# jayleicn/ClipBERT

Measured on NVIDIA H100. Metric: clips/sec fwd+bwd MSRVTT ret (ResNet50+BERT-base), higher is better.
Workload: dtype bf16

## Files before the change

clipbert_b200/csrc/gemm.cu:

```cuda
#include <algorithm>

#include "common.cuh"
#include "host_util.h"

namespace cb {

constexpr int BM = 128;
constexpr int BK = 64;
constexpr int CONSUMER_WARPS = 8;
constexpr int GEMM_THREADS = (CONSUMER_WARPS + 1) * 32;
constexpr int PP_THREADS = 3 * 128;
constexpr int PP_PRODUCER_REGS = 40;
constexpr int PP_CONSUMER_REGS = 232;
constexpr int PP_BAR_TURN = 1;
constexpr int MAX_STAGES = 8;
constexpr int SMEM_LIMIT = 232448;
constexpr int STG_PITCH = 36;
constexpr int STG_WARP_FLOATS = 16 * STG_PITCH;
constexpr int EPI_BYTES = CONSUMER_WARPS * STG_WARP_FLOATS * 4;
constexpr int IN_BOX_BYTES = BM * 64 * 2;

struct GemmEpi {
  const float* scale;
  const float* shift;
  const __nv_bfloat16* residual;
  const __nv_bfloat16* aux;
  int aux_mode;
  int act;
  void* out;
  int64_t out_ld;
  int out_fp32;
  __nv_bfloat16* out2;
  int64_t out2_ld;
  int rowmap, H, W;
  uint32_t drop_thresh;
// ... 179 lines not shown
        for (int j = 0; j < NC / 2; ++j) {
          const float2 a2 = unpack_bf16x2(aux16[j]);
          f[2 * j] *= a2.x;
          f[2 * j + 1] *= a2.y;
        }
        break;
      default: break;
    }
  }
}

struct TileInfo {
  int m0, n0;
};

template <int BN>
__device__ __forceinline__ TileInfo decode_tile(int tile, int tiles_m, int tiles_n) {
  TileInfo t;
  t.m0 = (tile / tiles_n) % tiles_m * BM;
  t.n0 = tile % tiles_n * BN;
  return t;
}

template <int BN, int TA, int TB>
__device__ __forceinline__ void mma_tile(float (&acc)[BN / 2], uint32_t smem0, int stage_bytes, int KCH, int STAGES, int n_iters, int wg,
                                         int lane, int& s, uint32_t& ph, uint64_t* full_bar, uint64_t* empty_bar) {
  using Cfg = GemmCfg<BN>;
  int prev = -1;
  for (int i = 0; i < n_iters; i += KCH) {
    const int nch = min(KCH, n_iters - i);
    mbar_wait(&full_bar[s], ph);
    __syncwarp();
    wgmma_fence();
    wgmma_fence_acc(acc);
    for (int ch = 0; ch < nch; ++ch) {
      const uint32_t a_addr = smem0 + s * stage_bytes + ch * Cfg::STAGE_BYTES + wg * (64 * 128);
      const uint32_t b_addr = smem0 + s * stage_bytes + ch * Cfg::STAGE_BYTES + Cfg::A_BYTES;
// ... 10 lines not shown
    if (prev >= 0) {
      __syncwarp();
      if (lane == 0) mbar_arrive(&empty_bar[prev]);
    }
    prev = s;
    if (++s == STAGES) { s = 0; ph ^= 1; }
  }
  wgmma_wait<0>();
  wgmma_fence_acc(acc);
  if (prev >= 0) {
    __syncwarp();
    if (lane == 0) mbar_arrive(&empty_bar[prev]);
  }
}

template <int BN, int TB>
__device__ __forceinline__ void mma_tile_pp(float (&acc)[2][BN / 2], uint32_t smem0, int stage_bytes, int KCH, int STAGES, int n_iters,
                                            int lane, int& s, uint32_t& ph, uint64_t* full_bar, uint64_t* empty_bar, int pass_bar,
                                            bool in_stage) {
  using Cfg = GemmCfg<BN>;
  int prev = -1;
  for (int i = 0; i < n_iters; i += KCH) {
    const int nch = min(KCH, n_iters - i);
    mbar_wait_unguarded(&full_bar[s], ph);
    __syncwarp();
    wgmma_fence();
    wgmma_fence_acc(acc[0]);
    wgmma_fence_acc(acc[1]);
    for (int ch = 0; ch < nch; ++ch) {
      const uint32_t a_addr = smem0 + s * stage_bytes + ch * Cfg::STAGE_BYTES;
      const uint32_t b_addr = a_addr + Cfg::A_BYTES;
#pragma unroll
      for (int k = 0; k < BK / 16; ++k) {
        const uint64_t bd = TB ? gmma_desc(b_addr + k * 2048, BK * 128, 1024) : gmma_desc(b_addr + k * 32, 16, 1024);
        const uint32_t accum = (i > 0 || ch > 0 || k > 0) ? 1u : 0u;
#pragma unroll
        for (int h = 0; h < 2; ++h) wgmma_bf16<BN, 0, TB>(acc[h], gmma_desc(a_addr + h * (64 * 128) + k * 32, 16, 1024), bd, accum);
      }
    }
    wgmma_commit();
    wgmma_wait<1>();
    wgmma_fence_acc(acc[0]);
    wgmma_fence_acc(acc[1]);
    if (prev >= 0) {
      __syncwarp();
      mbar_arrive_if(&empty_bar[prev], lane == 0);
// ... 25 lines not shown
    const int n = n0 + j * 8 + 2 * (lane & 3);
    if (n < N) {
      if constexpr (STORE) {
        if (r0 < M) *reinterpret_cast<float2*>(obase + static_cast<int64_t>(r0) * out_ld + n) = make_float2(acc[4 * j] * rs0, acc[4 * j + 1] * rs0);
        if (r1 < M) *reinterpret_cast<float2*>(obase + static_cast<int64_t>(r1) * out_ld + n) = make_float2(acc[4 * j + 2] * rs1, acc[4 * j + 3] * rs1);
      } else {
        if (r0 < M) red_add_f32x2(obase + static_cast<int64_t>(r0) * out_ld + n, acc[4 * j] * rs0, acc[4 * j + 1] * rs0);
        if (r1 < M) red_add_f32x2(obase + static_cast<int64_t>(r1) * out_ld + n, acc[4 * j + 2] * rs1, acc[4 * j + 3] * rs1);
      }
    }
  }
}

__device__ __forceinline__ uint32_t swz128(uint32_t box, int r, int q) { return box + r * 128 + ((q ^ (r & 7)) << 4); }

template <int BN, int MODE>
__global__ void __launch_bounds__(PP_THREADS, 1)
    gemm_pingpong_kernel(const __grid_constant__ CUtensorMap tmA, const __grid_constant__ CUtensorMap tmB, const __grid_constant__ CUtensorMap tmR,
                         const __grid_constant__ CUtensorMap tmX, int M, int N, int K, int ntaps, int tap_w, int tap_sign, int tiles_m,
                         int tiles_n, int total_tiles, int STAGES, int KCH, int N_IN, GemmEpi epi) {
  static_assert(MODE != 1 && BN <= 128, "TN / NN tiles of 128 x 64 or 128 x 128");
  using Cfg = GemmCfg<BN>;
  extern __shared__ uint8_t smem_raw[];
  uint8_t* smem = reinterpret_cast<uint8_t*>((reinterpret_cast<uintptr_t>(smem_raw) + 1023) & ~static_cast<uintptr_t>(1023));
  const int stage_bytes = KCH * Cfg::STAGE_BYTES;
  const bool has_res = epi.residual != nullptr, has_aux = epi.aux != nullptr;
  constexpr int IN_TILE_BYTES = (BN / 64) * IN_BOX_BYTES;
  const int in_bytes = (has_res + has_aux) * IN_TILE_BYTES;
  uint8_t* in_base = smem + STAGES * stage_bytes;
  uint8_t* stg_base = in_base + N_IN * in_bytes;
  uint64_t* full_bar = reinterpret_cast<uint64_t*>(stg_base + EPI_BYTES);
  uint64_t* empty_bar = full_bar + MAX_STAGES;
  uint64_t* in_full = empty_bar + MAX_STAGES;
  uint64_t* in_empty = in_full + 2;

  const int warp = __shfl_sync(0xffffffffu, static_cast<int>(threadIdx.x >> 5), 0);
  const int lane = threadIdx.x & 31;
  const int unit = blockIdx.x;
  const int n_units = gridDim.x;
  if (threadIdx.x == 0) dbg_stamp(epi, 0);
  pdl_trigger();
  if (threadIdx.x == 0) {
    tma_prefetch_desc(&tmA);
    tma_prefetch_desc(&tmB);
    if (has_res) tma_prefetch_desc(&tmR);
    if (has_aux) tma_prefetch_desc(&tmX);
    for (int s = 0; s < STAGES; ++s) {
      mbar_init(&full_bar[s], 1);
      mbar_init(&empty_bar[s], 4);
    }
    for (int b = 0; b < 2; ++b) {
      mbar_init(&in_full[b], 1);
      mbar_init(&in_empty[b], 4);
    }
    fence_mbar_init();
  }
  __syncthreads();
  const int kc_per_tap = (K + BK - 1) / BK;
  const int n_iters = ntaps * kc_per_tap;
  const bool in_stage = in_bytes && !N_IN;
  const int tile_stages = (n_iters + KCH - 1) / KCH + (in_stage ? 1 : 0);
  pdl_wait();
  if (threadIdx.x == 0) dbg_stamp(epi, 1);

  if (warp < 4) {
    setmaxnreg_dec<PP_PRODUCER_REGS>();
    if (warp == 0 && lane == 0) {
      constexpr int B_BOXES = (MODE == 0) ? 1 : BN / 64;
      int s = 0;
      uint32_t ph = 0;
      auto load_inputs = [&](int tile) {
        const TileInfo t = decode_tile<BN>(tile, tiles_m, tiles_n);
        uint64_t* bar;
        uint8_t* dst;
        if (N_IN) {
          const int local = (tile - unit) / n_units;
          const int b = N_IN == 2 ? (local & 1) : 0;
          const int uses = N_IN == 2 ? (local >> 1) : local;
          mbar_wait(&in_empty[b], (static_cast<uint32_t>(uses) & 1u) ^ 1u);
          bar = &in_full[local & 1];
          dst = in_base + b * in_bytes;
        } else {
          mbar_wait(&empty_bar[s], ph ^ 1);
          bar = &full_bar[s];
          dst = smem + s * stage_bytes;
          if (++s == STAGES) { s = 0; ph ^= 1; }
        }
        mbar_expect_tx(bar, in_bytes);
        if (has_res) {
#pragma unroll
          for (int j = 0; j < BN / 64; ++j) tma_load_2d(dst + j * IN_BOX_BYTES, &tmR, bar, t.n0 + j * 64, t.m0);
          dst += IN_TILE_BYTES;
        }
        if (has_aux) {
#pragma unroll
          for (int j = 0; j < BN / 64; ++j) tma_load_2d(dst + j * IN_BOX_BYTES, &tmX, bar, t.n0 + j * 64, t.m0);
        }
      };
      int pend = -1;
      for (int tile = unit; tile < total_tiles; tile += n_units) {
        const TileInfo t = decode_tile<BN>(tile, tiles_m, tiles_n);
        const bool inputs_first = tile < unit + N_IN * n_units;
        if (in_bytes && N_IN && inputs_first) load_inputs(tile);
        for (int i = 0; i < n_iters; i += KCH) {
          const int nch = min(KCH, n_iters - i);
          mbar_wait(&empty_bar[s], ph ^ 1);
          mbar_expect_tx(&full_bar[s], nch * Cfg::STAGE_BYTES);
          int tp = 0, kc = i;
          if (ntaps > 1) { tp = i / kc_per_tap; kc = i - tp * kc_per_tap; }
          for (int ch = 0; ch < nch; ++ch) {
            uint8_t* sa = smem + s * stage_bytes + ch * Cfg::STAGE_BYTES;
            uint8_t* sb = sa + Cfg::A_BYTES;
            int shift = 0;
            if (ntaps == 9) shift = tap_sign * ((tp / 3 - 1) * tap_w + (tp % 3 - 1));
            else if (ntaps > 1) shift = tap_sign * tp * tap_w;
            tma_load_2d(sa, &tmA, &full_bar[s], kc * BK, t.m0 + shift);
            if (MODE == 0) {
              tma_load_2d(sb, &tmB, &full_bar[s], tp * K + kc * BK, t.n0);
            } else if (epi.mn3d) {
              tma_load_3d(sb, &tmB, &full_bar[s], 0, kc * BK, (tp * N + t.n0) >> 6);
            } else {
#pragma unroll
              for (int j = 0; j < B_BOXES; ++j) tma_load_2d(sb + j * (BK * 128), &tmB, &full_bar[s], tp * N + t.n0 + j * 64, kc * BK);
            }
            if (++kc == kc_per_tap) { kc = 0; ++tp; }
          }
          if (++s == STAGES) { s = 0; ph ^= 1; }
          if (i == 0 && tile == unit) dbg_stamp(epi, 2);
        }
        if (in_stage) load_inputs(tile);
        if (pend >= 0) load_inputs(pend);
        pend = (in_bytes && N_IN && !inputs_first) ? tile : -1;
      }
      if (pend >= 0) load_inputs(pend);
      dbg_stamp(epi, 3);
    }
    return;
  }

  setmaxnreg_inc<PP_CONSUMER_REGS>();
  const int wg = (warp >> 2) - 1;
  const int wq = warp & 3;
  const uint32_t smem0 = smem_u32(smem);
  const uint64_t dseed = epi.drop_thresh ? drop_seed(epi.seed, epi.seed_off) : 0ull;
  float acc[2][BN / 2];
  int s = 0;
  uint32_t ph = 0;
  auto ring_skip = [&](int n) {
    s += n;
    while (s >= STAGES) { s -= STAGES; ph ^= 1; }
  };
  if (wg == 1) ring_skip(tile_stages);

  const int er = lane & 15, eh = lane >> 4;
  float* stg = reinterpret_cast<float*>(stg_base) + (warp - 4) * STG_WARP_FLOATS;
  const bool has_out2 = epi.out2 != nullptr;
  const bool has_shift = epi.shift != nullptr;
  const bool full = (N & 15) == 0 && epi.scale == nullptr;
  const bool drop = epi.drop_thresh != 0;
  int kind = EK_GENERIC;
  if (full) {
    if (!drop && !has_out2 && !has_aux && (epi.act == CB_ACT_NONE || epi.act == CB_ACT_RELU)) kind = EK_SHIFT_ACT;
    else if (!drop && !has_out2 && !has_shift && has_aux && epi.aux_mode == CB_AUX_RELU_MASK && epi.act == CB_ACT_NONE) kind = EK_RELU_MASK;
    else if (drop && !has_out2 && !has_aux && epi.act == CB_ACT_NONE) kind = EK_DROP_RES;
    else if (!drop && has_out2 && !has_aux && !has_res && epi.act == CB_ACT_GELU_STASH_GRAD) kind = EK_GELU_STASH;
    else if (!drop && !has_out2 && !has_shift && has_aux && epi.aux_mode == CB_AUX_MUL && epi.act == CB_ACT_NONE) kind = EK_AUX_MUL;
  }
  const bool kind_relu = epi.act == CB_ACT_RELU;
  const bool guard = (N & 15) != 0;

  for (int local = wg, tile = unit + wg * n_units; tile < total_tiles; local += 2, tile += 2 * n_units) {
    const TileInfo t = decode_tile<BN>(tile, tiles_m, tiles_n);
    if (local > 0) named_bar_sync(PP_BAR_TURN + wg, 2 * 128);
    const int pass = tile + n_units < total_tiles ? PP_BAR_TURN + (wg ^ 1) : 0;
    mma_tile_pp<BN, MODE != 0>(acc, smem0, stage_bytes, KCH, STAGES, n_iters, lane, s, ph, full_bar, empty_bar, pass, in_stage);

    const uint32_t in_buf = N_IN ? smem_u32(in_base) + (N_IN == 2 ? wg : 0) * in_bytes : smem0 + s * stage_bytes;
    if (in_bytes) {
      if (N_IN) mbar_wait_unguarded(&in_full[wg], static_cast<uint32_t>(local >> 1) & 1u);
      else mbar_wait_unguarded(&full_bar[s], ph);
    }
    int orow_half[2];
#pragma unroll
    for (int h = 0; h < 2; ++h) {
      const int m = t.m0 + h * 64 + wq * 16 + er;
      bool row_ok = m < M;
      int64_t orow = m;
      if (epi.rowmap == CB_ROWMAP_PAD) {
        const int hw = epi.H * epi.W;
        const int img = m / hw;
        const int r = m - img * hw;
        const int y = r / epi.W, x = r - y * epi.W;
        orow = (static_cast<int64_t>(img) * (epi.H + 2) + y + 1) * (epi.W + 2) + x + 1;
      } else if (epi.rowmap == CB_ROWMAP_UNPAD) {
        const int wp = epi.W + 2, hp = epi.H + 2;
// ... 25 lines not shown
        const int64_t orow = h ? orow_half[1] : orow_half[0];
        if (orow < 0 || nb >= N) continue;
        constexpr int NC = 16;
        float f[NC];
        const uint32_t srow = smem_u32(stg + er * STG_PITCH + eh * 16);
#pragma unroll
        for (int j = 0; j < NC / 4; ++j) {
          const uint4 u = lds128(srow + j * 16);
          f[4 * j] = __uint_as_float(u.x); f[4 * j + 1] = __uint_as_float(u.y);
          f[4 * j + 2] = __uint_as_float(u.z); f[4 * j + 3] = __uint_as_float(u.w);
        }
        uint32_t res16[NC / 2], aux16[NC / 2];
        const int tc = sc * 32 + eh * 16;
        const int q = (tc & 63) >> 3;
        if (has_res) {
#pragma unroll
          for (int j = 0; j < 2; ++j) {
            const uint4 u = lds128(swz128(in_buf + (tc >> 6) * IN_BOX_BYTES, wrow + er, q + j));
            res16[4 * j] = u.x; res16[4 * j + 1] = u.y; res16[4 * j + 2] = u.z; res16[4 * j + 3] = u.w;
          }
        }
        if (has_aux) {
#pragma unroll
          for (int j = 0; j < 2; ++j) {
            const uint4 u = lds128(swz128(in_buf + (has_res ? IN_TILE_BYTES : 0) + (tc >> 6) * IN_BOX_BYTES, wrow + er, q + j));
            aux16[4 * j] = u.x; aux16[4 * j + 1] = u.y; aux16[4 * j + 2] = u.z; aux16[4 * j + 3] = u.w;
          }
        }
        float shv[NC];
        if (has_shift) {
#pragma unroll
          for (int j = 0; j < NC; j += 4) {
            float4 s4 = make_float4(0.f, 0.f, 0.f, 0.f);
            if (nb + j + 4 <= N) s4 = __ldg(reinterpret_cast<const float4*>(epi.shift + nb + j));
            shv[j] = s4.x; shv[j + 1] = s4.y; shv[j + 2] = s4.z; shv[j + 3] = s4.w;
          }
        }
        uint32_t o2_16[NC / 2];
        switch (kind) {
          case EK_SHIFT_ACT: epilogue_shift_act<NC>(f, shv, has_shift, res16, has_res, kind_relu); break;
// ... 17 lines not shown
          __nv_bfloat16* o = reinterpret_cast<__nv_bfloat16*>(epi.out) + orow * epi.out_ld + nb;
#pragma unroll
          for (int j = 0; j < 2; ++j)
            if (nb + 8 * j + 8 <= N)
              *reinterpret_cast<uint4*>(o + 8 * j) = make_uint4(pack_bf16x2(f[8 * j], f[8 * j + 1]), pack_bf16x2(f[8 * j + 2], f[8 * j + 3]),
                                                                pack_bf16x2(f[8 * j + 4], f[8 * j + 5]), pack_bf16x2(f[8 * j + 6], f[8 * j + 7]));
        }
        if (has_out2) {
          __nv_bfloat16* o = epi.out2 + orow * epi.out2_ld + nb;
#pragma unroll
          for (int j = 0; j < 2; ++j)
            if (nb + 8 * j + 8 <= N) *reinterpret_cast<uint4*>(o + 8 * j) = make_uint4(o2_16[4 * j], o2_16[4 * j + 1], o2_16[4 * j + 2], o2_16[4 * j + 3]);
        }
      }
    }
    if (in_bytes) {
      __syncwarp();
      if (lane == 0) mbar_arrive(N_IN ? &in_empty[N_IN == 2 ? wg : 0] : &empty_bar[s]);
      if (!N_IN && ++s == STAGES) { s = 0; ph ^= 1; }
    }
    ring_skip(tile_stages);
  }
  if (threadIdx.x == 4 * 32) dbg_stamp(epi, 11);
}

static int g_sm_limit = 0;
static int sm_count_device() {
  static int n = 0;
  if (n == 0) {
    int dev = 0;
    cudaGetDevice(&dev);
    cudaDeviceGetAttribute(&n, cudaDevAttrMultiProcessorCount, dev);
    if (n <= 0) n = 132;
  }
  return n;
}
// ... 29 lines not shown
  const int stage_iters = ceil_div(kiters, p.kch);
  const int cap = staging ? 2 * stage_iters + 1 : (stage_iters + 1 > 2 ? stage_iters + 1 : 2);
  if (p.stages > cap) p.stages = cap;
  return p;
}
static SmemPlan plan_smem(int bn, bool staging, int kiters, int force_kch = 0, int in_bytes = 0) {
  const SmemPlan none = plan_ring(bn, staging, kiters, force_kch, 0, 0);
  if (in_bytes == 0) return none;
  const SmemPlan two = plan_ring(bn, staging, kiters, force_kch, in_bytes, 2);
  if (two.stages >= 2 && two.stages * two.kch >= kiters) return two;
  if (kiters > 4 && none.stages >= 2 && none.kch * none.chunk_bytes >= in_bytes) return none;
  return plan_ring(bn, staging, kiters, force_kch, in_bytes, 1);
}
static int epi_in_bytes(const cb_gemm_desc& d, int bn) {
  return d.mode == CB_GEMM_WGRAD ? 0 : ((d.residual != nullptr) + (d.aux != nullptr)) * (bn / 64) * IN_BOX_BYTES;
}

static int real_splits(int kc, int want) {
  const int sp = want < 1 ? 1 : (want > kc ? kc : want);
  return ceil_div(kc, ceil_div(kc, sp));
}

struct SplitReduceJob {
  float* out;
  const float* ws;
  int64_t out_ld;
  int M, W, S;
};
struct SplitReduce {
  int njobs;
// ... 14 lines not shown
    for (int s = 0; s < J.S; ++s) {
      const float4 a = *reinterpret_cast<const float4*>(p + s * plane);
      v.x += a.x; v.y += a.y; v.z += a.z; v.w += a.w;
    }
    *o = v;
  }
}
static int launch_split_reduce(const SplitReduce& r, cudaStream_t stream, const char* what) {
  int64_t most = 0;
  for (int i = 0; i < r.njobs; ++i) most = std::max(most, static_cast<int64_t>(r.j[i].M) * (r.j[i].W / 4));
  const int gx = static_cast<int>(std::min<int64_t>(1024, (most + 255) / 256));
  launch_k(wgrad_split_reduce_kernel, dim3(gx, r.njobs), 256, 0, stream, r);
  return check_launch(what);
}

template <int BN, int MODE>
static int launch_gemm(const cb_gemm_desc& d, const GemmEpi& epi_in, cudaStream_t stream) {
  GemmEpi epi = epi_in;
  using Cfg = GemmCfg<BN>;
  static bool attr_set = false;
  auto kern = gemm_pingpong_kernel<BN, MODE>;
  if (!attr_set) {
    cudaError_t e = cudaFuncSetAttribute(kern, cudaFuncAttributeMaxDynamicSharedMemorySize, SMEM_LIMIT);
    if (e != cudaSuccess) {
      set_error("cudaFuncSetAttribute(smem=%d): %s", SMEM_LIMIT, cudaGetErrorString(e));
      return CB_ERR_CUDA;
    }
    attr_set = true;
  }
  alignas(64) CUtensorMap ta, tb, tr, tx;
  bool mn3d = false;
  const int tiles_m = ceil_div(d.m, BM), tiles_n = ceil_div(d.n, BN);
  const int total = tiles_m * tiles_n;
  const int kiters = ceil_div(d.k, BK) * d.ntaps;
  bool ok = get_tmap_2d(&ta, d.a, d.k, d.a_rows, d.a_ld, BK, BM);
  if (MODE == 0) {
    ok = ok && get_tmap_2d(&tb, d.b, static_cast<uint64_t>(d.k) * d.ntaps, d.b_rows, d.b_ld, BK, BN);
  } else {
    mn3d = g_mn3d && d.n % 64 == 0 &&
           get_tmap_3d_mn(&tb, d.b, static_cast<uint64_t>(d.n) * d.ntaps, d.b_rows, d.b_ld, BK, BN / 64);
    if (!mn3d) ok = ok && get_tmap_2d(&tb, d.b, static_cast<uint64_t>(d.n) * d.ntaps, d.b_rows, d.b_ld, 64, BK);
  }
  tr = ta;
  tx = ta;
  if (d.residual) ok = ok && get_tmap_2d(&tr, d.residual, d.n, d.m, d.res_ld, 64, BM);
  if (d.aux) ok = ok && get_tmap_2d(&tx, d.aux, d.n, d.m, d.aux_ld, 64, BM);
  if (!ok) return CB_ERR_CUDA;
  epi.mn3d = mn3d ? 1 : 0;
  const int units = sm_count();
  const int grid = total < units ? total : units;
  const int in_bytes = epi_in_bytes(d, BN);
  const SmemPlan sp = plan_smem(BN, true, kiters, (d.reserved >> 8) & 15, in_bytes);
  const int kch = sp.kch, stages = sp.stages;
  if (stages < 2) {
    set_error("cb_gemm: not enough shared memory for a 2-stage pipeline (BN=%d, epilogue %d B + inputs %d B)", BN, sp.epi_bytes,
              in_bytes);
    return CB_ERR_INVALID;
  }
  const int smem_bytes = stages * kch * Cfg::STAGE_BYTES + sp.n_in * in_bytes + sp.epi_bytes + Cfg::BAR_BYTES + 1024;
  launch_gemm_k(kern, grid, PP_THREADS, smem_bytes, stream, ta, tb, tr, tx, d.m, d.n, d.k, d.ntaps, d.tap_w, d.tap_sign, tiles_m,
                tiles_n, total, stages, kch, sp.n_in, epi);
  return check_launch("cb_gemm");
}

struct LaunchCfg {
  int bn, splits;
};

static LaunchCfg choose_config(const cb_gemm_desc& d, int units) {
  const int kc = ceil_div(d.k, BK);
  const bool wgrad = d.mode == CB_GEMM_WGRAD;
  const int block_n = (!wgrad && d.block_n == 256) ? 128 : d.block_n;
  static const int cand[3] = {64, 128, 256};
  LaunchCfg best = {64, 1};
  double best_cost = 1e30;
  for (int c = 0; c < 3; ++c) {
    const int bn = cand[c];
    if (block_n && bn != block_n) continue;
    if (!wgrad && bn == 256) continue;
    if (bn > 64 && d.n <= bn / 2) continue;
    const int64_t base = static_cast<int64_t>(ceil_div(d.m, BM)) * ceil_div(d.n, bn) * (wgrad ? d.ntaps : 1);
    const int max_split = wgrad ? (d.split_k > 0 ? d.split_k : (kc < 32 ? kc : 32)) : 1;
    for (int sp = (wgrad && d.split_k > 0) ? d.split_k : 1; sp <= max_split; ++sp) {
      const int ips = ceil_div(wgrad ? kc : kc * d.ntaps, sp);
      const int real_sp = wgrad ? ceil_div(kc, ips) : 1;
      const int64_t tiles = base * real_sp;
      const double rounds = static_cast<double>((tiles + units - 1) / units);
      const SmemPlan pl = plan_smem(bn, !wgrad, ips, (d.reserved >> 8) & 15, epi_in_bytes(d, bn));
      if (pl.stages < 2) continue;
      const double shallow = (pl.stages * pl.kch < 3 && ips > 2) ? 3.0 : 1.0;
      const double stage_cost = 450.0 + pl.kch * pl.chunk_bytes / 60.0;
      const double main_loop = ceil_div(ips, pl.kch) * stage_cost * shallow;
      double cost;
      if (wgrad) {
        cost = rounds * (main_loop + bn * 24.0) + 2500.0;
      } else {
        const double epi = bn * 30.0;
        const double per_tile = main_loop > 0.5 * (main_loop + epi) ? main_loop : 0.5 * (main_loop + epi);
        cost = rounds * per_tile + 0.5 * epi + 2500.0;
      }
      if (cost < best_cost) {
        best_cost = cost;
        best = {bn, real_sp};
      }
    }
  }
  return best;
}

constexpr int WG_MAX_PROBLEMS = 8;
struct WgradProblem {
  CUtensorMap tmA, tmB;
  float* out;
  const float* scale;
  int64_t out_ld;
  int M, N, K;
  int ntaps, tap_w, tap_sign;
  int iters_per_split, tiles_m, tiles_n;
// ... 242 lines not shown
                         : launch_wgrad_group<64, false>(descs, n, splits, ws, stream, what);
    case 128: return need ? launch_wgrad_group<128, true>(descs, n, splits, ws, stream, what)
                          : launch_wgrad_group<128, false>(descs, n, splits, ws, stream, what);
    case 256: return need ? launch_wgrad_group<256, true>(descs, n, splits, ws, stream, what)
                          : launch_wgrad_group<256, false>(descs, n, splits, ws, stream, what);
    default: set_error("%s: block_n must be 0, 64, 128 or 256 (got %d)", what, bn); return CB_ERR_INVALID;
  }
}

}

extern "C" void cb_debug_gemm_timeline(void* device_buf) { cb::g_gemm_timeline = static_cast<long long*>(device_buf); }
extern "C" void cb_debug_gemm_mn3d(int on) { cb::g_mn3d = on ? 1 : 0; }
extern "C" void cb_debug_gemm_occ2(int, double) {}
extern "C" void cb_debug_gemm_sm_limit(int n) { cb::g_sm_limit = n > 0 ? n : 0; }

extern "C" int cb_gemm(const cb_gemm_desc* dp, void* stream_v) {
  using namespace cb;
  CB_REQUIRE(dp != nullptr, "cb_gemm: null descriptor");
  const cb_gemm_desc& d = *dp;
  cudaStream_t stream = static_cast<cudaStream_t>(stream_v);
  CB_REQUIRE(d.a && d.b && d.out, "cb_gemm: null operand pointer");
  CB_REQUIRE(d.m > 0 && d.n > 0 && d.k > 0, "cb_gemm: empty problem m=%d n=%d k=%d", d.m, d.n, d.k);
  CB_REQUIRE(d.ntaps == 1 || d.ntaps == 9 || (d.ntaps == 4 && d.mode == CB_GEMM_TN),
             "cb_gemm: ntaps must be 1, 9 (3x3 conv) or 4 (row taps, TN only) (got %d)", d.ntaps);
  CB_REQUIRE(d.mode == CB_GEMM_TN || d.mode == CB_GEMM_WGRAD || d.mode == CB_GEMM_NN, "cb_gemm: bad mode %d", d.mode);
  CB_REQUIRE(d.dropout_p >= 0.0f && d.dropout_p <= 1.0f, "cb_gemm: dropout_p %g outside [0, 1]", d.dropout_p);

  GemmEpi epi;
  epi.scale = d.scale;
// ... 24 lines not shown
    const bool nn = d.mode == CB_GEMM_NN;
    CB_REQUIRE(d.n % 8 == 0, "cb_gemm(TN): n must be a multiple of 8 (got %d)", d.n);
    CB_REQUIRE(d.k % 8 == 0, "cb_gemm(TN): k must be a multiple of 8 (got %d)", d.k);
    CB_REQUIRE(d.out_ld % 8 == 0, "cb_gemm(TN): out_ld must be a multiple of 8");
    CB_REQUIRE(!d.residual || d.res_ld % 8 == 0, "cb_gemm(TN): res_ld must be a multiple of 8");
    CB_REQUIRE(!d.aux || d.aux_ld % 8 == 0, "cb_gemm(TN): aux_ld must be a multiple of 8");
    CB_REQUIRE((reinterpret_cast<uintptr_t>(d.residual) & 15) == 0, "cb_gemm(TN): residual must be 16-byte aligned");
    CB_REQUIRE((reinterpret_cast<uintptr_t>(d.aux) & 15) == 0, "cb_gemm(TN): aux must be 16-byte aligned");
    CB_REQUIRE(!d.out2 || d.out2_ld % 8 == 0, "cb_gemm(TN): out2_ld must be a multiple of 8");
    CB_REQUIRE(!(d.out2 && d.out_fp32), "cb_gemm(TN): out2 requires a bf16 primary output");
    CB_REQUIRE(d.rowmap == CB_ROWMAP_NONE || (d.map_h > 0 && d.map_w > 0), "cb_gemm: rowmap needs map_h/map_w");
    CB_REQUIRE(d.ntaps == 1 || d.tap_w > 2, "cb_gemm: tap modes need tap_w (padded row pitch in pixels)");
    CB_REQUIRE(d.block_n == 0 || d.block_n == 64 || d.block_n == 128 || d.block_n == 256, "cb_gemm: block_n must be 0, 64, 128 or 256 (got %d)",
               d.block_n);
    const LaunchCfg lc = choose_config(d, sm_count());
    switch (lc.bn) {
      case 64: return nn ? launch_gemm<64, 2>(d, epi, stream) : launch_gemm<64, 0>(d, epi, stream);
      case 128: return nn ? launch_gemm<128, 2>(d, epi, stream) : launch_gemm<128, 0>(d, epi, stream);
      default: CB_REQUIRE(false, "cb_gemm: no tile width for block_n %d", d.block_n);
    }
  } else {
    const int rc = check_wgrad_desc(d, "cb_gemm(WGRAD)");
    if (rc != CB_OK) return rc;
    const LaunchCfg lc = choose_config(d, plan_sm_count());
    return launch_wgrad(&d, 1, lc.bn, lc.splits, stream, "cb_gemm");
  }
  return CB_ERR_INVALID;
}

extern "C" int cb_gemm_wgrad_group(const cb_gemm_desc* descs, int n, void* stream_v) {
// ... 36 lines not shown
```

clipbert_b200/ops.py:

```python
import ctypes

import torch

from . import _lib as L
from ._lib import (ACT_GELU, ACT_GELU_STASH_GRAD, ACT_NONE, ACT_RELU, ACT_TANH, AUX_GELU_GRAD, AUX_MUL, AUX_NONE,
                   AUX_RELU_MASK, AUX_TANH_GRAD, CB_GEMM_TN, CB_GEMM_WGRAD, ROWMAP_NONE, ROWMAP_PAD, ROWMAP_UNPAD)

CB_GEMM_NN = 2
_c = ctypes
_vp, _i, _i64, _f, _u64 = _c.c_void_p, _c.c_int, _c.c_int64, _c.c_float, _c.c_uint64

_SIGS = {
    "cb_layernorm_fwd": [_vp, _vp, _vp, _vp, _vp, _i, _i, _f, _vp],
    "cb_layernorm_bwd": [_vp, _vp, _vp, _vp, _vp, _vp, _vp, _vp, _vp, _i, _i, _f, _u64, _vp],
    "cb_embed_text_fwd": [_vp, _vp, _vp, _vp, _vp, _vp, _vp, _vp, _i, _i, _i, _i, _i, _f, _f, _u64, _vp],
    "cb_embed_text_bwd": [_vp] * 12 + [_i, _i, _i, _i, _i, _f, _u64, _vp],
    "cb_embed_visual_fwd": [_vp, _vp, _i, _vp, _vp, _vp, _vp, _vp, _vp, _vp, _i, _i, _i, _i, _i, _i, _i, _f, _f, _u64, _vp],
    "cb_embed_visual_bwd": [_vp, _vp, _vp, _vp, _i] + [_vp] * 12 + [_i, _i, _i, _i, _i, _i, _i, _i, _f, _u64, _vp],
    "cb_colsum": [_vp, _i64, _vp, _i, _i, _vp],
    "cb_dropout": [_vp, _vp, _i64, _f, _u64, _vp],
    "cb_dropout_offset_advance": [_vp, _vp, _vp],
    "cb_gelu_bwd": [_vp, _vp, _vp, _i64, _vp],
    "cb_pad_cast": [_vp, _i64, _vp, _i, _i, _i, _vp],
    "cb_cast_scale": [_vp, _vp, _i64, _vp, _i64, _vp],
# ... 98 lines not shown
    f.restype = None
    f(int(mode), float(max_gflop))


def dropout_offset_bind(word):
    f = L.lib().cb_dropout_offset_bind
    f.argtypes = [_vp]
    f.restype = _c.c_int
    f(None if word is None else word.data_ptr())


def dropout_offset_advance(counter, snapshot=None):
    _call("cb_dropout_offset_advance", _p(counter), _p(snapshot), _s())


def set_sm_limit(n):
    L.lib().cb_debug_gemm_sm_limit(int(n))


def set_pdl(enable):
    return int(L.lib().cb_set_pdl(2 if int(enable) == 2 else int(bool(enable))))


_lib_deterministic = False


def set_deterministic(on):
    return bool(L.lib().cb_set_deterministic(int(bool(on))))


# ... 136 lines not shown
            d = arr[0]
            label = ("gemm mode=%d m=%d n=%d k=%d taps=%d res=%d aux=%d o2=%d f32=%d rm=%d" % (
                d.mode, d.m, d.n, d.k, d.ntaps, bool(d.residual), bool(d.aux), bool(d.out2), d.out_fp32, d.rowmap)
                if name == "cb_gemm" else "gemm wgrad group x%d" % len(kws))
            _op_timing.append((label, e0, e1))


def gemm(**kw):
    if _tuning is None:
        _load_tuning()
    if _gemm_record is not None:
        _gemm_record.append(dict(kw))
    if _tuning and "block_n" not in kw and "reserved" not in kw:
        t = _tuning.get(gemm_key(kw))
        if t is not None:
            kw = dict(kw, block_n=t[0], split_k=t[1], reserved=(t[2] << 8) | (32 if (len(t) > 3 and t[3]) else 0))
    if kw.get("mode", CB_GEMM_TN) == CB_GEMM_WGRAD and deterministic():
        kw = _with_workspace(kw, gemm_workspace_bytes(kw))
    _launch_gemm("cb_gemm", [kw])


group_wgrad = 3


def gemm_wgrad_group(kws):
    if not kws:
        return
    if len(kws) == 1:
        for kw in kws:
            gemm(**kw)
        return
# ... 228 lines not shown
```

include/clipbert_b200.h:

```cpp
#ifndef CLIPBERT_B200_H_
#define CLIPBERT_B200_H_

#include <stddef.h>
#include <stdint.h>

#ifdef __cplusplus
extern "C" {
#endif

typedef enum cb_status {
  CB_OK = 0,
  CB_ERR_INVALID = -1,
  CB_ERR_CUDA = -2,
  CB_ERR_UNSUPPORTED = -3
} cb_status;

const char* cb_last_error(void);
int cb_version(void);
int cb_sm_arch(void);
int64_t cb_launch_count(void);
int cb_set_pdl(int enable);

int cb_set_deterministic(int enable);

// ... 37 lines not shown
  int32_t act;
  void* out;
  int64_t out_ld;
  int32_t out_fp32;
  void* out2;
  int64_t out2_ld;
  int32_t rowmap, map_h, map_w;
  float dropout_p;
  uint64_t dropout_seed;
  int32_t block_n;
  int32_t reserved;
  void* workspace;
  int64_t workspace_bytes;
} cb_gemm_desc;

int cb_gemm(const cb_gemm_desc* desc, void* stream);
int64_t cb_gemm_workspace_bytes(const cb_gemm_desc* desc);
int cb_gemm_wgrad_group(const cb_gemm_desc* descs, int n, void* stream);
int64_t cb_gemm_wgrad_group_workspace_bytes(const cb_gemm_desc* descs, int n);

int cb_layernorm_fwd(const void* x, const float* gamma, const float* beta, void* y, float* stats, int m, int hidden,
                     float eps, void* stream);
int cb_layernorm_bwd(const void* dy, const void* x, const float* stats, const float* gamma, void* dx, void* dx_drop,
                     float* dgamma, float* dbeta, float* dbias_drop, int m, int hidden, float dropout_p,
                     uint64_t dropout_seed, void* stream);
int64_t cb_layernorm_bwd_scratch_bytes(int m);
int cb_layernorm_bwd_det(const void* dy, const void* x, const float* stats, const float* gamma, void* dx, void* dx_drop,
                         float* dgamma, float* dbeta, float* dbias_drop, int m, int hidden, float dropout_p,
                         uint64_t dropout_seed, float* scratch, int64_t scratch_bytes, void* stream);

int cb_embed_text_fwd(const int64_t* ids, const float* word, const float* pos, const float* type0, const float* gamma,
// ... 87 lines not shown
```

Baseline: 3978.

## Add cooperative paired 256-wide tiles to the ping-pong TN/NN GEMM

Adds a paired mode to the ping-pong GEMM kernel in which both consumer warpgroups work on one 256x128 or 128x256 tile at the same time, each handling one 128x128 half. The A or B operand is shared in shared memory, which cuts operand traffic per output. The ping-pong alternation is dropped in this mode and residual and aux inputs are staged through the main ring. A cost model in choose_config picks between paired and unpaired tiles, and a tuning flag can force 256-row tiles. The risk is losing the overlap of one warpgroup's epilogue with the other's main loop, and a less flexible shared-memory layout.

```diff
diff --git a/clipbert_b200/csrc/gemm.cu b/clipbert_b200/csrc/gemm.cu
--- a/clipbert_b200/csrc/gemm.cu
+++ b/clipbert_b200/csrc/gemm.cu
@@ -19,6 +19,7 @@
 constexpr int STG_WARP_FLOATS = 16 * STG_PITCH;
 constexpr int EPI_BYTES = CONSUMER_WARPS * STG_WARP_FLOATS * 4;
 constexpr int IN_BOX_BYTES = BM * 64 * 2;
+constexpr double PAIRED_B_PER_CLK = 60.0;
 
 struct GemmEpi {
   const float* scale;
@@ -228,13 +229,22 @@
   int m0, n0;
 };
 
-template <int BN>
+template <int TM, int TN>
 __device__ __forceinline__ TileInfo decode_tile(int tile, int tiles_m, int tiles_n) {
   TileInfo t;
-  t.m0 = (tile / tiles_n) % tiles_m * BM;
-  t.n0 = tile % tiles_n * BN;
+  t.m0 = (tile / tiles_n) % tiles_m * TM;
+  t.n0 = tile % tiles_n * TN;
   return t;
 }
+
+enum { PAIR_NONE = 0, PAIR_N = 1, PAIR_M = 2 };
+template <int BN, int PAIR>
+struct PairCfg {
+  static constexpr int TM = PAIR == PAIR_M ? 2 * BM : BM;
+  static constexpr int TN = PAIR == PAIR_N ? 2 * BN : BN;
+  static constexpr int A_BYTES = TM * BK * 2;
+  static constexpr int CHUNK_BYTES = (TM + TN) * BK * 2;
+};
 
 template <int BN, int TA, int TB>
 __device__ __forceinline__ void mma_tile(float (&acc)[BN / 2], uint32_t smem0, int stage_bytes, int KCH, int STAGES, int n_iters, int wg,
@@ -275,11 +285,17 @@
   }
 }
 
-template <int BN, int TB>
-__device__ __forceinline__ void mma_tile_pp(float (&acc)[2][BN / 2], uint32_t smem0, int stage_bytes, int KCH, int STAGES, int n_iters,
-                                            int lane, int& s, uint32_t& ph, uint64_t* full_bar, uint64_t* empty_bar, int pass_bar,
-                                            bool in_stage) {
+__device__ __forceinline__ int pp_consumer() {
+  uint32_t tid;
+  asm volatile("mov.u32 %0, %%tid.x;" : "=r"(tid));
+  return static_cast<int>(tid >> 7) - 1;
+}
+template <int BN, int TB, int PAIR = PAIR_NONE>
+__device__ __forceinline__ void mma_tile_pp(float (&acc)[2][BN / 2], uint32_t smem0, int stage_bytes, int KCH, int STAGES,
+                                            int n_iters, int lane, int& s, uint32_t& ph, uint64_t* full_bar, uint64_t* empty_bar,
+                                            int pass_bar, bool in_stage) {
   using Cfg = GemmCfg<BN>;
+  using PCfg = PairCfg<BN, PAIR>;
   int prev = -1;
   for (int i = 0; i < n_iters; i += KCH) {
     const int nch = min(KCH, n_iters - i);
@@ -288,9 +304,11 @@
     wgmma_fence();
     wgmma_fence_acc(acc[0]);
     wgmma_fence_acc(acc[1]);
+    const int half = PAIR != PAIR_NONE ? pp_consumer() : 0;
     for (int ch = 0; ch < nch; ++ch) {
-      const uint32_t a_addr = smem0 + s * stage_bytes + ch * Cfg::STAGE_BYTES;
-      const uint32_t b_addr = a_addr + Cfg::A_BYTES;
+      const uint32_t c_addr = smem0 + s * stage_bytes + ch * PCfg::CHUNK_BYTES;
+      const uint32_t a_addr = c_addr + (PAIR == PAIR_M ? half * Cfg::A_BYTES : 0);
+      const uint32_t b_addr = c_addr + PCfg::A_BYTES + (PAIR == PAIR_N ? half * Cfg::B_BYTES : 0);
 #pragma unroll
       for (int k = 0; k < BK / 16; ++k) {
         const uint64_t bd = TB ? gmma_desc(b_addr + k * 2048, BK * 128, 1024) : gmma_desc(b_addr + k * 32, 16, 1024);
@@ -346,16 +364,19 @@
 
 __device__ __forceinline__ uint32_t swz128(uint32_t box, int r, int q) { return box + r * 128 + ((q ^ (r & 7)) << 4); }
 
-template <int BN, int MODE>
+template <int BN, int MODE, int PAIR = PAIR_NONE>
 __global__ void __launch_bounds__(PP_THREADS, 1)
     gemm_pingpong_kernel(const __grid_constant__ CUtensorMap tmA, const __grid_constant__ CUtensorMap tmB, const __grid_constant__ CUtensorMap tmR,
                          const __grid_constant__ CUtensorMap tmX, int M, int N, int K, int ntaps, int tap_w, int tap_sign, int tiles_m,
                          int tiles_n, int total_tiles, int STAGES, int KCH, int N_IN, GemmEpi epi) {
   static_assert(MODE != 1 && BN <= 128, "TN / NN tiles of 128 x 64 or 128 x 128");
+  static_assert(PAIR == PAIR_NONE || BN == 128, "paired tiles are two 128 x 128 halves");
   using Cfg = GemmCfg<BN>;
+  using PCfg = PairCfg<BN, PAIR>;
+  if constexpr (PAIR != PAIR_NONE) N_IN = 0;
   extern __shared__ uint8_t smem_raw[];
   uint8_t* smem = reinterpret_cast<uint8_t*>((reinterpret_cast<uintptr_t>(smem_raw) + 1023) & ~static_cast<uintptr_t>(1023));
-  const int stage_bytes = KCH * Cfg::STAGE_BYTES;
+  const int stage_bytes = KCH * PCfg::CHUNK_BYTES;
   const bool has_res = epi.residual != nullptr, has_aux = epi.aux != nullptr;
   constexpr int IN_TILE_BYTES = (BN / 64) * IN_BOX_BYTES;
   const int in_bytes = (has_res + has_aux) * IN_TILE_BYTES;
@@ -379,7 +400,7 @@
     if (has_aux) tma_prefetch_desc(&tmX);
     for (int s = 0; s < STAGES; ++s) {
       mbar_init(&full_bar[s], 1);
-      mbar_init(&empty_bar[s], 4);
+      mbar_init(&empty_bar[s], PAIR ? 8 : 4);
     }
     for (int b = 0; b < 2; ++b) {
       mbar_init(&in_full[b], 1);
@@ -390,7 +411,7 @@
   __syncthreads();
   const int kc_per_tap = (K + BK - 1) / BK;
   const int n_iters = ntaps * kc_per_tap;
-  const bool in_stage = in_bytes && !N_IN;
+  const bool in_stage = PAIR == PAIR_NONE && in_bytes && !N_IN;
   const int tile_stages = (n_iters + KCH - 1) / KCH + (in_stage ? 1 : 0);
   pdl_wait();
   if (threadIdx.x == 0) dbg_stamp(epi, 1);
@@ -398,11 +419,11 @@
   if (warp < 4) {
     setmaxnreg_dec<PP_PRODUCER_REGS>();
     if (warp == 0 && lane == 0) {
-      constexpr int B_BOXES = (MODE == 0) ? 1 : BN / 64;
+      constexpr int B_BOXES = (MODE == 0) ? PCfg::TN / BN : PCfg::TN / 64;
       int s = 0;
       uint32_t ph = 0;
       auto load_inputs = [&](int tile) {
-        const TileInfo t = decode_tile<BN>(tile, tiles_m, tiles_n);
+        const TileInfo t = decode_tile<BM, BN>(tile, tiles_m, tiles_n);
         uint64_t* bar;
         uint8_t* dst;
         if (N_IN) {
@@ -429,26 +450,35 @@
           for (int j = 0; j < BN / 64; ++j) tma_load_2d(dst + j * IN_BOX_BYTES, &tmX, bar, t.n0 + j * 64, t.m0);
         }
       };
+      auto load_input_stage = [&](const CUtensorMap* tm, int m0, int n0) {
+        mbar_wait(&empty_bar[s], ph ^ 1);
+        mbar_expect_tx(&full_bar[s], IN_TILE_BYTES);
+#pragma unroll
+        for (int j = 0; j < BN / 64; ++j) tma_load_2d(smem + s * stage_bytes + j * IN_BOX_BYTES, tm, &full_bar[s], n0 + j * 64, m0);
+        if (++s == STAGES) { s = 0; ph ^= 1; }
+      };
       int pend = -1;
       for (int tile = unit; tile < total_tiles; tile += n_units) {
-        const TileInfo t = decode_tile<BN>(tile, tiles_m, tiles_n);
+        const TileInfo t = decode_tile<PCfg::TM, PCfg::TN>(tile, tiles_m, tiles_n);
         const bool inputs_first = tile < unit + N_IN * n_units;
         if (in_bytes && N_IN && inputs_first) load_inputs(tile);
         for (int i = 0; i < n_iters; i += KCH) {
           const int nch = min(KCH, n_iters - i);
           mbar_wait(&empty_bar[s], ph ^ 1);
-          mbar_expect_tx(&full_bar[s], nch * Cfg::STAGE_BYTES);
+          mbar_expect_tx(&full_bar[s], nch * PCfg::CHUNK_BYTES);
           int tp = 0, kc = i;
           if (ntaps > 1) { tp = i / kc_per_tap; kc = i - tp * kc_per_tap; }
           for (int ch = 0; ch < nch; ++ch) {
-            uint8_t* sa = smem + s * stage_bytes + ch * Cfg::STAGE_BYTES;
-            uint8_t* sb = sa + Cfg::A_BYTES;
+            uint8_t* sa = smem + s * stage_bytes + ch * PCfg::CHUNK_BYTES;
+            uint8_t* sb = sa + PCfg::A_BYTES;
             int shift = 0;
             if (ntaps == 9) shift = tap_sign * ((tp / 3 - 1) * tap_w + (tp % 3 - 1));
             else if (ntaps > 1) shift = tap_sign * tp * tap_w;
-            tma_load_2d(sa, &tmA, &full_bar[s], kc * BK, t.m0 + shift);
+#pragma unroll
+            for (int j = 0; j < PCfg::TM / BM; ++j) tma_load_2d(sa + j * Cfg::A_BYTES, &tmA, &full_bar[s], kc * BK, t.m0 + j * BM + shift);
             if (MODE == 0) {
-              tma_load_2d(sb, &tmB, &full_bar[s], tp * K + kc * BK, t.n0);
+#pragma unroll
+              for (int j = 0; j < B_BOXES; ++j) tma_load_2d(sb + j * Cfg::B_BYTES, &tmB, &full_bar[s], tp * K + kc * BK, t.n0 + j * BN);
             } else if (epi.mn3d) {
               tma_load_3d(sb, &tmB, &full_bar[s], 0, kc * BK, (tp * N + t.n0) >> 6);
             } else {
@@ -459,6 +489,14 @@
           }
           if (++s == STAGES) { s = 0; ph ^= 1; }
           if (i == 0 && tile == unit) dbg_stamp(epi, 2);
+        }
+        if constexpr (PAIR != PAIR_NONE) {
+#pragma unroll
+          for (int c = 0; c < 2; ++c) {
+            const int m0 = t.m0 + (PAIR == PAIR_M ? c * BM : 0), n0 = t.n0 + (PAIR == PAIR_N ? c * BN : 0);
+            if (has_res) load_input_stage(&tmR, m0, n0);
+            if (has_aux) load_input_stage(&tmX, m0, n0);
+          }
         }
         if (in_stage) load_inputs(tile);
         if (pend >= 0) load_inputs(pend);
@@ -482,7 +520,8 @@
     s += n;
     while (s >= STAGES) { s -= STAGES; ph ^= 1; }
   };
-  if (wg == 1) ring_skip(tile_stages);
+  if (PAIR == PAIR_NONE && wg == 1) ring_skip(tile_stages);
+  const int n_inputs = has_res + has_aux;
 
   const int er = lane & 15, eh = lane >> 4;
   float* stg = reinterpret_cast<float*>(stg_base) + (warp - 4) * STG_WARP_FLOATS;
@@ -501,16 +540,34 @@
   const bool kind_relu = epi.act == CB_ACT_RELU;
   const bool guard = (N & 15) != 0;
 
-  for (int local = wg, tile = unit + wg * n_units; tile < total_tiles; local += 2, tile += 2 * n_units) {
-    const TileInfo t = decode_tile<BN>(tile, tiles_m, tiles_n);
-    if (local > 0) named_bar_sync(PP_BAR_TURN + wg, 2 * 128);
-    const int pass = tile + n_units < total_tiles ? PP_BAR_TURN + (wg ^ 1) : 0;
-    mma_tile_pp<BN, MODE != 0>(acc, smem0, stage_bytes, KCH, STAGES, n_iters, lane, s, ph, full_bar, empty_bar, pass, in_stage);
-
-    const uint32_t in_buf = N_IN ? smem_u32(in_base) + (N_IN == 2 ? wg : 0) * in_bytes : smem0 + s * stage_bytes;
-    if (in_bytes) {
-      if (N_IN) mbar_wait_unguarded(&in_full[wg], static_cast<uint32_t>(local >> 1) & 1u);
-      else mbar_wait_unguarded(&full_bar[s], ph);
+  constexpr int TSTEP = PAIR == PAIR_NONE ? 2 : 1;
+  for (int local = PAIR == PAIR_NONE ? wg : 0, tile = unit + local * n_units; tile < total_tiles; local += TSTEP, tile += TSTEP * n_units) {
+    TileInfo t = decode_tile<PCfg::TM, PCfg::TN>(tile, tiles_m, tiles_n);
+    if (PAIR == PAIR_M) t.m0 += pp_consumer() * BM;
+    if (PAIR == PAIR_N) t.n0 += pp_consumer() * BN;
+    if (PAIR == PAIR_NONE && local > 0) named_bar_sync(PP_BAR_TURN + wg, 2 * 128);
+    const int pass = PAIR == PAIR_NONE && tile + n_units < total_tiles ? PP_BAR_TURN + (wg ^ 1) : 0;
+    mma_tile_pp<BN, MODE != 0, PAIR>(acc, smem0, stage_bytes, KCH, STAGES, n_iters, lane, s, ph, full_bar, empty_bar, pass, in_stage);
+
+    auto input_stage = [&](int j) {
+      int si = s + wg * n_inputs + j;
+      while (si >= STAGES) si -= STAGES;
+      return smem0 + si * stage_bytes;
+    };
+    uint32_t in_buf = 0;
+    if constexpr (PAIR != PAIR_NONE) {
+      int si = s;
+      uint32_t pi = ph;
+      for (int j = 0; j < (wg + 1) * n_inputs; ++j) {
+        if (j >= wg * n_inputs) mbar_wait_unguarded(&full_bar[si], pi);
+        if (++si == STAGES) { si = 0; pi ^= 1; }
+      }
+    } else {
+      in_buf = N_IN ? smem_u32(in_base) + (N_IN == 2 ? wg : 0) * in_bytes : smem0 + s * stage_bytes;
+      if (in_bytes) {
+        if (N_IN) mbar_wait_unguarded(&in_full[wg], static_cast<uint32_t>(local >> 1) & 1u);
+        else mbar_wait_unguarded(&full_bar[s], ph);
+      }
     }
     int orow_half[2];
 #pragma unroll
@@ -566,16 +623,18 @@
         const int tc = sc * 32 + eh * 16;
         const int q = (tc & 63) >> 3;
         if (has_res) {
+          const uint32_t res_buf = PAIR != PAIR_NONE ? input_stage(0) : in_buf;
 #pragma unroll
           for (int j = 0; j < 2; ++j) {
-            const uint4 u = lds128(swz128(in_buf + (tc >> 6) * IN_BOX_BYTES, wrow + er, q + j));
+            const uint4 u = lds128(swz128(res_buf + (tc >> 6) * IN_BOX_BYTES, wrow + er, q + j));
             res16[4 * j] = u.x; res16[4 * j + 1] = u.y; res16[4 * j + 2] = u.z; res16[4 * j + 3] = u.w;
           }
         }
         if (has_aux) {
+          const uint32_t aux_buf = PAIR != PAIR_NONE ? input_stage(has_res) : in_buf + (has_res ? IN_TILE_BYTES : 0);
 #pragma unroll
           for (int j = 0; j < 2; ++j) {
-            const uint4 u = lds128(swz128(in_buf + (has_res ? IN_TILE_BYTES : 0) + (tc >> 6) * IN_BOX_BYTES, wrow + er, q + j));
+            const uint4 u = lds128(swz128(aux_buf + (tc >> 6) * IN_BOX_BYTES, wrow + er, q + j));
             aux16[4 * j] = u.x; aux16[4 * j + 1] = u.y; aux16[4 * j + 2] = u.z; aux16[4 * j + 3] = u.w;
           }
         }
@@ -623,12 +682,21 @@
         }
       }
     }
-    if (in_bytes) {
-      __syncwarp();
-      if (lane == 0) mbar_arrive(N_IN ? &in_empty[N_IN == 2 ? wg : 0] : &empty_bar[s]);
-      if (!N_IN && ++s == STAGES) { s = 0; ph ^= 1; }
-    }
-    ring_skip(tile_stages);
+    if constexpr (PAIR != PAIR_NONE) {
+      for (int j = 0; j < 2 * n_inputs; ++j) {
+        mbar_wait_unguarded(&full_bar[s], ph);
+        __syncwarp();
+        if (lane == 0) mbar_arrive(&empty_bar[s]);
+        if (++s == STAGES) { s = 0; ph ^= 1; }
+      }
+    } else {
+      if (in_bytes) {
+        __syncwarp();
+        if (lane == 0) mbar_arrive(N_IN ? &in_empty[N_IN == 2 ? wg : 0] : &empty_bar[s]);
+        if (!N_IN && ++s == STAGES) { s = 0; ph ^= 1; }
+      }
+      ring_skip(tile_stages);
+    }
   }
   if (threadIdx.x == 4 * 32) dbg_stamp(epi, 11);
 }
@@ -688,6 +756,17 @@
 }
 static int epi_in_bytes(const cb_gemm_desc& d, int bn) {
   return d.mode == CB_GEMM_WGRAD ? 0 : ((d.residual != nullptr) + (d.aux != nullptr)) * (bn / 64) * IN_BOX_BYTES;
+}
+static SmemPlan plan_tn(const cb_gemm_desc& d, int bn, bool paired, int kiters) {
+  const int force_kch = (d.reserved >> 8) & 15;
+  if (!paired) return plan_smem(bn, true, kiters, force_kch, epi_in_bytes(d, bn));
+  SmemPlan p = plan_ring(2 * bn, true, kiters, force_kch ? force_kch : 1, 0, 0);
+  const int need = 2 * ((d.residual != nullptr) + (d.aux != nullptr));
+  if (p.stages < need) {
+    const int fit = std::min(MAX_STAGES, (SMEM_LIMIT - 1024 - GemmCfg<64>::BAR_BYTES - p.epi_bytes) / (p.kch * p.chunk_bytes));
+    p.stages = fit >= need ? need : 0;
+  }
+  return p;
 }
 
 static int real_splits(int kc, int want) {
@@ -732,12 +811,12 @@
   return check_launch(what);
 }
 
-template <int BN, int MODE>
+template <int BN, int MODE, int PAIR = PAIR_NONE>
 static int launch_gemm(const cb_gemm_desc& d, const GemmEpi& epi_in, cudaStream_t stream) {
   GemmEpi epi = epi_in;
-  using Cfg = GemmCfg<BN>;
+  using PCfg = PairCfg<BN, PAIR>;
   static bool attr_set = false;
-  auto kern = gemm_pingpong_kernel<BN, MODE>;
+  auto kern = gemm_pingpong_kernel<BN, MODE, PAIR>;
   if (!attr_set) {
     cudaError_t e = cudaFuncSetAttribute(kern, cudaFuncAttributeMaxDynamicSharedMemorySize, SMEM_LIMIT);
     if (e != cudaSuccess) {
@@ -748,7 +827,7 @@
   }
   alignas(64) CUtensorMap ta, tb, tr, tx;
   bool mn3d = false;
-  const int tiles_m = ceil_div(d.m, BM), tiles_n = ceil_div(d.n, BN);
+  const int tiles_m = ceil_div(d.m, PCfg::TM), tiles_n = ceil_div(d.n, PCfg::TN);
   const int total = tiles_m * tiles_n;
   const int kiters = ceil_div(d.k, BK) * d.ntaps;
   bool ok = get_tmap_2d(&ta, d.a, d.k, d.a_rows, d.a_ld, BK, BM);
@@ -756,7 +835,7 @@
     ok = ok && get_tmap_2d(&tb, d.b, static_cast<uint64_t>(d.k) * d.ntaps, d.b_rows, d.b_ld, BK, BN);
   } else {
     mn3d = g_mn3d && d.n % 64 == 0 &&
-           get_tmap_3d_mn(&tb, d.b, static_cast<uint64_t>(d.n) * d.ntaps, d.b_rows, d.b_ld, BK, BN / 64);
+           get_tmap_3d_mn(&tb, d.b, static_cast<uint64_t>(d.n) * d.ntaps, d.b_rows, d.b_ld, BK, PCfg::TN / 64);
     if (!mn3d) ok = ok && get_tmap_2d(&tb, d.b, static_cast<uint64_t>(d.n) * d.ntaps, d.b_rows, d.b_ld, 64, BK);
   }
   tr = ta;
@@ -768,14 +847,14 @@
   const int units = sm_count();
   const int grid = total < units ? total : units;
   const int in_bytes = epi_in_bytes(d, BN);
-  const SmemPlan sp = plan_smem(BN, true, kiters, (d.reserved >> 8) & 15, in_bytes);
+  const SmemPlan sp = plan_tn(d, BN, PAIR != PAIR_NONE, kiters);
   const int kch = sp.kch, stages = sp.stages;
   if (stages < 2) {
     set_error("cb_gemm: not enough shared memory for a 2-stage pipeline (BN=%d, epilogue %d B + inputs %d B)", BN, sp.epi_bytes,
               in_bytes);
     return CB_ERR_INVALID;
   }
-  const int smem_bytes = stages * kch * Cfg::STAGE_BYTES + sp.n_in * in_bytes + sp.epi_bytes + Cfg::BAR_BYTES + 1024;
+  const int smem_bytes = stages * kch * PCfg::CHUNK_BYTES + sp.n_in * in_bytes + sp.epi_bytes + GemmCfg<BN>::BAR_BYTES + 1024;
   launch_gemm_k(kern, grid, PP_THREADS, smem_bytes, stream, ta, tb, tr, tx, d.m, d.n, d.k, d.ntaps, d.tap_w, d.tap_sign, tiles_m,
                 tiles_n, total, stages, kch, sp.n_in, epi);
   return check_launch("cb_gemm");
@@ -783,35 +862,42 @@
 
 struct LaunchCfg {
   int bn, splits;
+  int pair;
 };
 
 static LaunchCfg choose_config(const cb_gemm_desc& d, int units) {
   const int kc = ceil_div(d.k, BK);
   const bool wgrad = d.mode == CB_GEMM_WGRAD;
-  const int block_n = (!wgrad && d.block_n == 256) ? 128 : d.block_n;
-  static const int cand[3] = {64, 128, 256};
-  LaunchCfg best = {64, 1};
+  static const LaunchCfg tn_cand[4] = {{64, 1, PAIR_NONE}, {128, 1, PAIR_NONE}, {128, 1, PAIR_N}, {128, 1, PAIR_M}};
+  static const LaunchCfg wg_cand[3] = {{64, 1, PAIR_NONE}, {128, 1, PAIR_NONE}, {256, 1, PAIR_NONE}};
+  const bool rows256 = !wgrad && (d.reserved & CB_GEMM_TILE_256_ROWS);
+  LaunchCfg best = {64, 1, PAIR_NONE};
   double best_cost = 1e30;
-  for (int c = 0; c < 3; ++c) {
-    const int bn = cand[c];
-    if (block_n && bn != block_n) continue;
-    if (!wgrad && bn == 256) continue;
-    if (bn > 64 && d.n <= bn / 2) continue;
-    const int64_t base = static_cast<int64_t>(ceil_div(d.m, BM)) * ceil_div(d.n, bn) * (wgrad ? d.ntaps : 1);
+  for (int c = 0; c < (wgrad ? 3 : 4); ++c) {
+    const LaunchCfg cc = wgrad ? wg_cand[c] : tn_cand[c];
+    const int bn = cc.bn;
+    const bool paired = cc.pair != PAIR_NONE;
+    const int tile_m = cc.pair == PAIR_M ? 2 * BM : BM, tile_n = cc.pair == PAIR_N ? 2 * bn : bn;
+    if (rows256 ? cc.pair != PAIR_M : d.block_n && (tile_n != d.block_n || cc.pair == PAIR_M)) continue;
+    if (tile_n > 64 && d.n <= tile_n / 2) continue;
+    if (tile_m > BM && d.m <= BM) continue;
+    const int64_t base = static_cast<int64_t>(ceil_div(d.m, tile_m)) * ceil_div(d.n, tile_n) * (wgrad ? d.ntaps : 1);
     const int max_split = wgrad ? (d.split_k > 0 ? d.split_k : (kc < 32 ? kc : 32)) : 1;
     for (int sp = (wgrad && d.split_k > 0) ? d.split_k : 1; sp <= max_split; ++sp) {
       const int ips = ceil_div(wgrad ? kc : kc * d.ntaps, sp);
       const int real_sp = wgrad ? ceil_div(kc, ips) : 1;
       const int64_t tiles = base * real_sp;
       const double rounds = static_cast<double>((tiles + units - 1) / units);
-      const SmemPlan pl = plan_smem(bn, !wgrad, ips, (d.reserved >> 8) & 15, epi_in_bytes(d, bn));
+      const SmemPlan pl = wgrad ? plan_smem(bn, false, ips, (d.reserved >> 8) & 15) : plan_tn(d, bn, paired, ips);
       if (pl.stages < 2) continue;
       const double shallow = (pl.stages * pl.kch < 3 && ips > 2) ? 3.0 : 1.0;
-      const double stage_cost = 450.0 + pl.kch * pl.chunk_bytes / 60.0;
+      const double stage_cost = 450.0 + pl.kch * pl.chunk_bytes / (paired ? PAIRED_B_PER_CLK : 60.0);
       const double main_loop = ceil_div(ips, pl.kch) * stage_cost * shallow;
       double cost;
       if (wgrad) {
         cost = rounds * (main_loop + bn * 24.0) + 2500.0;
+      } else if (paired) {
+        cost = rounds * (main_loop + bn * 30.0) + 2500.0;
       } else {
         const double epi = bn * 30.0;
         const double per_tile = main_loop > 0.5 * (main_loop + epi) ? main_loop : 0.5 * (main_loop + epi);
@@ -819,7 +905,7 @@
       }
       if (cost < best_cost) {
         best_cost = cost;
-        best = {bn, real_sp};
+        best = {bn, real_sp, cc.pair};
       }
     }
   }
@@ -1092,6 +1178,12 @@
 extern "C" void cb_debug_gemm_mn3d(int on) { cb::g_mn3d = on ? 1 : 0; }
 extern "C" void cb_debug_gemm_occ2(int, double) {}
 extern "C" void cb_debug_gemm_sm_limit(int n) { cb::g_sm_limit = n > 0 ? n : 0; }
+extern "C" int cb_gemm_tile(const cb_gemm_desc* d) {
+  using namespace cb;
+  if (d == nullptr || (d->mode != CB_GEMM_TN && d->mode != CB_GEMM_NN) || d->m <= 0 || d->n <= 0 || d->k <= 0) return 0;
+  const LaunchCfg lc = choose_config(*d, sm_count());
+  return ((lc.pair == PAIR_M ? 2 * BM : BM) << 16) | (lc.pair == PAIR_N ? 2 * lc.bn : lc.bn);
+}
 
 extern "C" int cb_gemm(const cb_gemm_desc* dp, void* stream_v) {
   using namespace cb;
@@ -1146,6 +1238,8 @@
     CB_REQUIRE(d.block_n == 0 || d.block_n == 64 || d.block_n == 128 || d.block_n == 256, "cb_gemm: block_n must be 0, 64, 128 or 256 (got %d)",
                d.block_n);
     const LaunchCfg lc = choose_config(d, sm_count());
+    if (lc.pair == PAIR_N) return nn ? launch_gemm<128, 2, PAIR_N>(d, epi, stream) : launch_gemm<128, 0, PAIR_N>(d, epi, stream);
+    if (lc.pair == PAIR_M) return nn ? launch_gemm<128, 2, PAIR_M>(d, epi, stream) : launch_gemm<128, 0, PAIR_M>(d, epi, stream);
     switch (lc.bn) {
       case 64: return nn ? launch_gemm<64, 2>(d, epi, stream) : launch_gemm<64, 0>(d, epi, stream);
       case 128: return nn ? launch_gemm<128, 2>(d, epi, stream) : launch_gemm<128, 0>(d, epi, stream);
diff --git a/clipbert_b200/ops.py b/clipbert_b200/ops.py
--- a/clipbert_b200/ops.py
+++ b/clipbert_b200/ops.py
@@ -7,6 +7,7 @@
                    AUX_RELU_MASK, AUX_TANH_GRAD, CB_GEMM_TN, CB_GEMM_WGRAD, ROWMAP_NONE, ROWMAP_PAD, ROWMAP_UNPAD)
 
 CB_GEMM_NN = 2
+CB_GEMM_TILE_256_ROWS = 16
 _c = ctypes
 _vp, _i, _i64, _f, _u64 = _c.c_void_p, _c.c_int, _c.c_int64, _c.c_float, _c.c_uint64
 
@@ -136,6 +137,14 @@
     _call("cb_dropout_offset_advance", _p(counter), _p(snapshot), _s())
 
 
+def gemm_tile(**kw):
+    f = L.lib().cb_gemm_tile
+    f.argtypes = [_c.POINTER(L.GemmDesc)]
+    f.restype = _c.c_int
+    v = f(_gemm_descs([kw]))
+    return (v >> 16, v & 0xFFFF) if v else None
+
+
 def set_sm_limit(n):
     L.lib().cb_debug_gemm_sm_limit(int(n))
 
@@ -302,7 +311,8 @@
     if _tuning and "block_n" not in kw and "reserved" not in kw:
         t = _tuning.get(gemm_key(kw))
         if t is not None:
-            kw = dict(kw, block_n=t[0], split_k=t[1], reserved=(t[2] << 8) | (32 if (len(t) > 3 and t[3]) else 0))
+            kw = dict(kw, block_n=t[0], split_k=t[1],
+                      reserved=(t[2] << 8) | (32 if (len(t) > 3 and t[3]) else 0) | (CB_GEMM_TILE_256_ROWS if (len(t) > 4 and t[4]) else 0))
     if kw.get("mode", CB_GEMM_TN) == CB_GEMM_WGRAD and deterministic():
         kw = _with_workspace(kw, gemm_workspace_bytes(kw))
     _launch_gemm("cb_gemm", [kw])
diff --git a/include/clipbert_b200.h b/include/clipbert_b200.h
--- a/include/clipbert_b200.h
+++ b/include/clipbert_b200.h
@@ -75,7 +75,10 @@
   int64_t workspace_bytes;
 } cb_gemm_desc;
 
+enum { CB_GEMM_TILE_256_ROWS = 16 };
+
 int cb_gemm(const cb_gemm_desc* desc, void* stream);
+int cb_gemm_tile(const cb_gemm_desc* desc);
 int64_t cb_gemm_workspace_bytes(const cb_gemm_desc* desc);
 int cb_gemm_wgrad_group(const cb_gemm_desc* descs, int n, void* stream);
 int64_t cb_gemm_wgrad_group_workspace_bytes(const cb_gemm_desc* descs, int n);
```

New measurement: 4081 (median of 6 runs). 1.03x the previous value.
